# fusiyuan2010/CSC

Hardware: AMD Instinct MI355X
Metric: encode MB/s (10^6 input bytes / wall-clock) on enwik9 stand-in, -m3 -d64m; stream bit-exact vs reference (higher is better)
Workload: dtype u8/u32 (byte + 32-bit integer work; 12-bit probabilities, 64-bit range-coder low)

## Files before the change

### csc_amd/csrc/csc_host.cpp

```cpp
#include <hip/hip_runtime.h>
#include <chrono>

#include <math.h>
#include <stdio.h>
#include <stdlib.h>
#include <string.h>

#include <mutex>
#include <vector>

#include "../../include/csc_mi355x.h"
#include "csc_device.h"
#include "csc_enc_frame.h"
#include "csc_tables.h"

namespace cscmi {
hipError_t upload_tables();
void launch_frame_blocks(const FrameItem *items, FrameJob *jobs, FrameStatus *status, uint32_t nstreams, hipStream_t st);
void launch_init_state(EncState *S, hipStream_t st);
void launch_analyze(EncState *S, uint32_t chunk_size, const double *ent_coef, hipStream_t st);
void launch_encode_runs(int parser, EncState *S, const RunDesc *runs, uint32_t nruns, uint32_t reset_arena, hipStream_t st);
void launch_encode_eof(EncState *S, hipStream_t st);
void launch_encode_runs_multi(int parser, uint32_t nstreams, EncState *const *states, const RunDesc *const *runs,
                              const uint32_t *nruns, const uint32_t *reset, hipStream_t st);
// ... 1008 lines not shown
    HIPCHK(hipStreamSynchronize(e->stream));
    if (result) *result = e->h_small[0];
    return 0;
}
int CSCST_SetPos(CSCEncHandle p, uint32_t pos)
{
    EncInstance *e = (EncInstance *)p;
    if (!e) return -1;
    HIPCHK(hipSetDevice(e->device));
    HIPCHK(hipStreamSynchronize(e->stream));
    HIPCHK(hipMemcpy(&e->d_state->pos, &pos, sizeof(pos), hipMemcpyHostToDevice));
    return 0;
}
#endif

#ifdef CSCMI_TIMERS
void CSCMI_DebugTimers(CSCEncHandle p, uint64_t *out16)
{
    EncInstance *e = (EncInstance *)p;
    KernelStats ks;
    memset(&ks, 0, sizeof(ks));
    (void)hipSetDevice(e->device);
    (void)hipMemcpy(&ks, &e->d_state->stats, sizeof(ks), hipMemcpyDeviceToHost);
    for (int i = 0; i < 16; i++) out16[i] = ks.tm[i];
}

void CSCMI_DebugSetMask(CSCEncHandle p, uint64_t mask)
{
    EncInstance *e = (EncInstance *)p;
    (void)hipSetDevice(e->device);
    (void)hipMemcpy(&e->d_state->stats.trace[63][0], &mask, sizeof(mask), hipMemcpyHostToDevice);
}

void CSCMI_DebugTrace(CSCEncHandle p, uint64_t *out768)
{
    EncInstance *e = (EncInstance *)p;
    static KernelStats ks;
    memset(&ks, 0, sizeof(ks));
    (void)hipSetDevice(e->device);
    (void)hipMemcpy(&ks, &e->d_state->stats, sizeof(ks), hipMemcpyDeviceToHost);
    memcpy(out768, ks.trace, sizeof(ks.trace));
}
#endif

}
```

### csc_amd/csrc/csc_kernels_dp4.inc

```

constexpr uint32_t kD4Rec = 256;
constexpr uint32_t kD4CandEnt = kD4Rec * 4;
constexpr uint32_t kD4RefEnt = 256;
constexpr uint32_t kD4Ent = kD4CandEnt + kD4RefEnt;
constexpr uint32_t kD4LA = 48;
constexpr uint32_t kD4Waves = 12;
DEV uint32_t d4_role(uint32_t w)
{
    constexpr uint32_t roles[12] = { 0, 6, 7, 1, 8, 5, 4, 2, 8, 8, 9, 3 };
    return w < 12 ? roles[w] : 8u;
}
constexpr uint32_t kD4Requested = 0xFFFFFFFFu;
#ifndef D4_IDLE_MUL
#define D4_IDLE_MUL 1
#endif
constexpr int kD4IdleSleep = 4 * D4_IDLE_MUL;
constexpr uint32_t kD4RefreshAt = 32;
constexpr uint32_t kD4MaxGood = 16;
constexpr uint32_t kD6Ring = 128;
constexpr uint32_t kD6MRing = 64;
constexpr uint32_t kD4MultiMax = 768;

struct Dp4X {
    uint32_t sb_seq, sb_ack, quit, abort;
    uint32_t sb0, pos0, size, gen;
    uint32_t m_pos;
    uint32_t m_ids[2];
    uint32_t ins_head;
    uint32_t cmp_next, cmp_pause, cmp_idle[3], cmp_cur[3];
    uint32_t ev_seq, ev_s, ev_len, ev_ack;
    uint32_t ref_head;
    uint32_t rq_head, rq_tail;
    uint32_t lit_req, lit_from, lit_done;
    uint32_t rid[4];
    uint32_t io_w0, io_gen, io_state0, io_lp_int, io_lit_seq, io_rq_head, io_wnd_lo, io_wnd_hi, io_wnd_size, io_vld, io_good, io_plit_lo, io_plit_hi;
    alignas(16) uint32_t o_kind, o_end, o_a0l, o_a0code, o_a0eid, o_a0slot, o_fin_i0, o_fin_i1, o_lp_int, o_lit_seq, o_rq_head, o_err;
#ifdef CSCMI_TIMERS
    uint32_t stat[8];
    uint32_t wtm[52];
#endif
    uint32_t rq[16][2];
    raw_vec4 cand[kD4Rec];
    uint8_t hflag[kD4Rec];
    uint32_t rec_tag[kD4Rec], rec_hsum[kD4Rec], rec_a0d[kD4Rec], rec_len[kD4Rec][16];
    uint32_t rec_m32[kD4Rec][16];
    raw_vec4 ent[kD4Ent];
    uint32_t fwd[kD4Ent];
    alignas(512) uint16_t litp[4][kD4Rec];
    alignas(16) uint16_t tab[64][32];
    alignas(256) raw_vec4 lab[16];
    alignas(512) uint32_t tent[2][16][8];
    alignas(256) raw_vec4 ver[16];
    uint32_t lab_seq, win_seq;
    alignas(16) uint32_t dump[8];
    alignas(8) uint32_t e_prog[2]; uint32_t e_stop[2];
#ifdef CSCMI_TIMERS
    uint32_t dbgp[64], dbgq[64][8], dbgl[32];
    uint32_t dbg;
    uint32_t tr_win, tr_lo, tr_hi;
#endif
    uint32_t lenp_new[32];
    uint32_t lt_pub, lt_done;
    uint32_t lt_rec[kD6Ring];
    uint32_t mt_pub, mt_done;
    uint32_t mt_rec[kD6MRing][2];
    uint32_t hS[2], h_reset, hand[20];
};
struct EncLds4 { EncLds base; Dp4X x; CoderQ q; };
__shared__ EncLds4 g_lds4;

DEV uint32_t d4_tag(uint32_t gen, uint32_t p) { return ((gen << 13) | p) + 1u; }
DEV Dp4X *d4x(Sc &c) { return reinterpret_cast<Dp4X *>(c.X); }

DEV uint32_t d4_eq4(uint32_t x)
{
    const uint32_t z = ~(((x & 0x7F7F7F7Fu) + 0x7F7F7F7Fu) | x) & 0x80808080u;
    return (((z >> 7) * 0x01020408u) >> 24) & 0xFu;
}
DEV uint32_t d4_eq8(uint64_t x) { return d4_eq4((uint32_t)x) | (d4_eq4((uint32_t)(x >> 32)) << 4); }

DEV bool d4_spin(Sc &c, Dp4X *X, uint32_t &spins, uint32_t site)
{
    __builtin_amdgcn_s_sleep(1);
    if ((++spins & 1023u) == 0 && (spins > (kDpSpinLimit << 2) || lds_vload(&X->abort))) {
        if (!lds_vload(&X->abort)) lds_vstore(&X->abort, 0x40000000u | (site << 16) | (c.wv << 24) | (spins & 0xFFFFu));
        c.error = lds_vload(&X->abort);
        return false;
    }
    return true;
}
template <int LANE> DEV uint32_t d4_wrlane(uint32_t old, uint32_t val)
{
// ... 1128 lines not shown
        if (__ballot(ask) != 0) rq_head = UNI(d4_ask(__ballot(ask), rid_v, wpos, rq_head));
        if (__ballot(arrived) != 0) { lds_fence(); if (arrived) rid_v = fwv - 1; }
        const bool hard = lane < 4 && !arrived && age >= kD5HardAge && age < 0x80000000u;
        if (__builtin_expect(__ballot(hard) == 0, 1)) break;
        __builtin_amdgcn_s_sleep(1);
#ifdef CSCMI_TIMERS
        if (spins == 0 && lane == 0) atomicAdd(&X->stat[7], 1u);
#endif
        if ((++spins & 4095u) == 0 && (UNI(*(lds_vu32 *)&X->abort) || spins > (kDpSpinLimit << 2))) {
            if (!UNI(*(lds_vu32 *)&X->abort)) *(lds_vu32 *)&X->abort = 0x40100000u | (spins & 0xFFFFu);
            break;
        }
    }
    raw_vec4 r;
    r.x = rdlane(rid_v, 0) | (rdlane(rid_v, 1) << 16); r.y = rdlane(rid_v, 2) | (rdlane(rid_v, 3) << 16); r.z = rq_head; r.w = 0;
    return r;
}

__device__ __noinline__ void d5_spine()
{
    EncLds *L = &g_lds4.base;
    Dp4X *X = &g_lds4.x;
    const uint32_t lane = threadIdx.x & 63u;
    const uint32_t sb0 = UNI(X->sb0), size = UNI(X->size);
    const uint32_t w0 = UNI(X->io_w0), good = UNI(X->io_good);
    uint32_t lit_seq = UNI(X->io_lit_seq), rq_head = UNI(X->io_rq_head);
    const uint32_t aplimit = umin(kAPLimit, size - w0);
    const uint32_t sel_rid = lane < 4 ? 0x0C0C0100u + lane * 0x0202u : 0x0C0C0C0Cu;
#ifdef CSCMI_TIMERS
    const unsigned long long tsp = __builtin_readcyclecounter();
    unsigned long long t_first = 0, t_poll = 0, t_gen = 0, t_last = 0;
    uint32_t n_gen = 0;
#endif
    dp_fence();
    lit_seq++;
    d5_lit_guard(lit_seq);
    *(lds_vu32 *)&X->lit_from = umin(w0 + 8u, size);
    lds_fence();
    *(lds_vu32 *)&X->lit_req = lit_seq;
    uint32_t own_p = 0, own_bit = 0;
    const uint32_t own_pos = w0 + (lane >> 3);
    {
        const gu32 *p_lit = (const gu32 *)(((uint64_t)UNI(X->io_plit_hi) << 32) | UNI(X->io_plit_lo));
        const uint32_t b01 = (uint32_t)stage_load8(L->stage, umin(own_pos, size) + 15u);
        const uint32_t ctx = (sb0 + own_pos) ? (b01 & 0xFFu) : 0u, cc = ((b01 >> 8) & 0xFFu) | 0x100u;
        const uint32_t j = lane & 7u;
        own_bit = (cc >> (7u - j)) & 1u;
        if (own_pos < size) own_p = p_lit[ctx * 256u + (cc >> (8u - j))];
    }
    {
        const uint32_t lastwin = UNI(*(lds_vu32 *)&X->win_seq);
        uint32_t spins = 0;
        while (!(lds_vload(&X->e_stop[0]) == lastwin && lds_vload(&X->e_stop[1]) == lastwin)) {
            if ((++spins & 4095u) == 0 && (lds_vload(&X->abort) || spins > (kDpSpinLimit << 2))) { if (!lds_vload(&X->abort)) *(lds_vu32 *)&X->abort = 0x400F0000u; break; }
        }
        lds_fence();
    }
    d4_build_tables_inl();
    {
        uint32_t pr = L->p2b[(own_bit ? own_p : 4096u - own_p) >> 3];
        pr += (uint32_t)__shfl_xor((int)pr, 1);
        pr += (uint32_t)__shfl_xor((int)pr, 2);
        pr += (uint32_t)__shfl_xor((int)pr, 4);
        if ((lane & 7u) == 0 && own_pos < size) X->litp[lit_seq & 3u][own_pos & (kD4Rec - 1)] = (uint16_t)pr;
        lds_fence();
    }
    const uint32_t own_upto = w0 + 8u;
    uint32_t vz;
    asm volatile("v_mov_b32 %0, 0" : "=v"(vz));
    uint32_t vP = vz, vD = vz, vBS = (UNI(X->io_state0) << 16) | vz;
    uint32_t vI0, vI1;
    {
        uint32_t i0 = UNI(X->rid[0]) | (UNI(X->rid[1]) << 16), i1 = UNI(X->rid[2]) | (UNI(X->rid[3]) << 16);
        d5_forward_ids(X, lane, sel_rid, i0, i1);
        vI0 = i0 | vz; vI1 = i1 | vz;
    }
    uint32_t v_lp = UNI(X->io_lp_int) | vz, v_reach = vz;
    uint32_t refreshed = 0, have_new = 0;
    {
        const uint32_t lp0 = UNI(v_lp);
        if (lp0 < 96u) { d6_wait_match_trees(); d4_len_price_rebuild(X->lenp_new); have_new = 1; }
        raw_vec4 lb;
        lb.x = vP; lb.y = vBS | (lp0 < kD5Zone2 ? (lp0 + 1u) << 24 : 0u); lb.z = vI0; lb.w = vI1;
        *(lds_vvec4 *)&X->lab[0] = lb;
    }
    *(lds_vu32 *)&X->tent[0][1][0] = kD5Inf; *(lds_vu32 *)&X->tent[1][1][0] = kD5Inf; *(lds_vu32 *)&X->tent[1][2][0] = kD5Inf;
    { raw_vec4 z; z.x = z.y = z.z = z.w = 0; *(lds_vvec4 *)&X->ver[15] = z; }
    lds_fence();
    *(lds_vu32 *)&X->lab_seq = 1;
    const uint32_t win = UNI(*(lds_vu32 *)&X->win_seq) + 1u;
    const uint32_t winhi = (win & 0xFFFFu) << 16;
    lds_fence();
    *(lds_vu32 *)&X->win_seq = win;
#ifdef CSCMI_TIMERS
    const unsigned long long ts0 = __builtin_readcyclecounter();
    uint32_t n_straight = 0;
    unsigned long long *const TR = (unsigned long long *)(((uint64_t)UNI(X->tr_hi) << 32) | UNI(X->tr_lo));
    const bool tr_on = win == UNI(X->tr_win);
#endif
    uint32_t k = 0, kind = DP_CONT, end = 0, vnext = 0, lit_ok = own_upto, err = 0;
    uint32_t a0l = 1, a0code = 0, a0eid = 0, a0slot = 0, fI0 = 0, fI1 = 0;
    typedef volatile __attribute__((address_space(3))) uint8_t lds_vu8;
    const uint32_t f7 = lane & 7u, l16 = lane & 15u;
    const uint32_t mP = f7 == D5F_P ? ~0u : 0u, mBS = f7 == D5F_BS ? ~0u : 0u, mD = f7 == D5F_D ? ~0u : 0u, mTBV = f7 == D5F_TBV ? ~0u : 0u;
    const uint32_t shv = f7 == D5F_M32 ? 1u : 0u;
    const uint32_t c_left = f7 == D5F_LEFT ? ~0u : 0u;
    const uint32_t m_lsign = f7 == D5F_LEFT ? 0x80000000u : 0u;
    const uint32_t mlow = f7 == D5F_BS ? 0xFFFFu : ~0u;
    const uint32_t mI0 = f7 == D5F_I0 ? ~0u : 0u, mI1 = f7 == D5F_I1 ? ~0u : 0u, mM32 = f7 == D5F_M32 ? ~0u : 0u;
    auto lbl_pack = [&](uint32_t P, uint32_t D, uint32_t BS, uint32_t I0, uint32_t I1, uint32_t TBV, uint32_t M32, uint32_t LEFT) -> uint32_t {
        return (P & mP) | (BS & mBS) | (D & mD) | (I0 & mI0) | (I1 & mI1) | (TBV & mTBV) | (M32 & mM32) | (LEFT & c_left);
    };
    const uint32_t m_lab = 0u - ((0x001Bu >> l16) & 1u), m_log = 0u - ((0x0204u >> l16) & 1u);
    const uint32_t a_img = (uint32_t)(uintptr_t)(lds_vu8 *)&g_lds4;
    const uint32_t a_lab = a_img + (((uint32_t)(uintptr_t)(lds_vu8 *)&X->lab[0] - a_img) & m_lab);
    auto lds_at = [](uint32_t a) { return (lds_vu32 *)(uintptr_t)a; };
    static_assert(sizeof(((Dp4X *)nullptr)->lab) == 256 && sizeof(((Dp4X *)nullptr)->dump) >= 32, "label ring of 16 x 16 bytes (the store offset wraps at 256); eight dump words");
    const uint32_t r_log0 = (uint32_t)(uintptr_t)(lds_vu8 *)&L->fin2[0] - a_img, r_dump = (uint32_t)(uintptr_t)(lds_vu8 *)&X->dump[0] - a_img;
    const uint32_t st_inc = (16u & m_lab) | (8u & m_log);
    const uint32_t st_and = 255u | ~m_lab;
    const uint32_t w_lab = ((0x32010u >> (l16 * 4u)) & 0xFu) * 4u;
    const uint32_t w_log = (l16 >> 3) * 4u;
    auto st_seek = [&](uint32_t kk) -> uint32_t {
        const uint32_t o_lab = (kk & 15u) * 16u + w_lab, o_log = r_log0 + kk * 8u + w_log, o_dmp = r_dump + f7 * 4u;
        return (o_lab & m_lab) | (o_log & m_log) | (o_dmp & ~(m_lab | m_log));
    };
    uint64_t prog = 0;
    raw_vec4 V;
    uint32_t T0 = 0, T1 = 0, tree = 0;
    V.x = V.y = V.z = V.w = 0;
    static_assert(sizeof(((Dp4X *)nullptr)->ver) == 256 && sizeof(((Dp4X *)nullptr)->tent[0]) == 512 && sizeof(((Dp4X *)nullptr)->litp[0]) == 512, "ring sizes the address wraps assume");
    const uint32_t a_ver0 = (uint32_t)(uintptr_t)(lds_vu8 *)&X->ver[0], a_tent0 = (uint32_t)(uintptr_t)(lds_vu8 *)&X->tent[0][0][0];
    const uint32_t a_litp0 = (uint32_t)(uintptr_t)(lds_vu8 *)&X->litp[lit_seq & 3u][0];
// ... 316 lines not shown
                    bP = UNI(A.x); bBS = UNI(A.y); bD = UNI(A.z); bI0 = UNI(A.w); bI1 = UNI(*(lds_vu32 *)&X->tent[t & 1u][t & 15u][4]);
                }
                if (k >= 2) {
                    const raw_vec4 B = *(lds_vvec4 *)&X->tent[k & 1u][t & 15u][0];
                    const uint32_t qP = UNI(B.x), qBS = UNI(B.y), qD = UNI(B.z), qI0 = UNI(B.w), qI1 = UNI(*(lds_vu32 *)&X->tent[k & 1u][t & 15u][4]);
                    if (qP < bP || (qP == bP && (qBS & 0xFFFFu) < (bBS & 0xFFFFu))) { bP = qP; bD = qD; bBS = qBS; bI0 = qI0; bI1 = qI1; }
                }
                if (eP < bP) { bP = eP; bD = eD; bBS = eBS; bI0 = cI0; bI1 = cI1; }
                cP = bP; cD = bD; cBS = bBS; cI0 = bI0; cI1 = bI1;
                k++;
                raw_vec4 lb;
                lb.x = cP; lb.y = cBS | (refreshed << 31) | (lp_int < kD5Zone2 ? (lp_int + 1u) << 24 : 0u); lb.z = cI0; lb.w = cI1;
                *(lds_vvec4 *)&X->lab[k & 15u] = lb;
                L->fin2[k * 2u] = cD; L->fin2[k * 2u + 1u] = cBS;
#ifdef CSCMI_TIMERS
                if (k < 64) { X->dbgq[k][0] = cP; X->dbgq[k][5] = eP; X->dbgq[k][6] = 2; X->dbgq[k][7] = lp_int; }
#endif
                lds_fence();
                *(lds_vu32 *)&X->lab_seq = k + 1u;
            }
            vP = cP | vz; vD = cD | vz; vBS = cBS | vz; vI0 = cI0 | vz; vI1 = cI1 | vz; v_lp = lp_int | vz; v_reach = reach | vz;
            fI0 = cI0; fI1 = cI1;
            if (!out) pf_label();
#ifdef CSCMI_TIMERS
            t_gen += __builtin_readcyclecounter() - tg0;
#endif
            if (out) break;
        }
    }
#ifdef CSCMI_TIMERS
    const unsigned long long tse = __builtin_readcyclecounter();
    if (lane == 0) { atomicAdd(&X->wtm[13], (uint32_t)(tse - ts0) >> 4); atomicAdd(&X->wtm[14], n_straight); atomicAdd(&X->wtm[15], 1u);
        atomicAdd(&X->wtm[24], (uint32_t)(ts0 - tsp) >> 4); atomicAdd(&X->wtm[25], (uint32_t)t_first >> 4); atomicAdd(&X->wtm[26], (uint32_t)t_poll >> 4);
        atomicAdd(&X->wtm[27], (uint32_t)t_gen >> 4); atomicAdd(&X->wtm[28], n_gen); atomicAdd(&X->wtm[29], (uint32_t)(tse - t_last) >> 4); }
#endif
    lds_fence();
    *(lds_vu32 *)&X->lab_seq = kD5Stop;
    if (refreshed) { if (lane < 32) L->len_price[lane] = X->lenp_new[lane]; lds_fence(); }
    uint32_t f0 = kind == DP_EXIT_LIMIT ? fI0 : UNI(X->lab[end & 15u].z);
    uint32_t f1 = kind == DP_EXIT_LIMIT ? fI1 : UNI(X->lab[end & 15u].w);
    d5_forward_ids(X, lane, sel_rid, f0, f1);
    *(lds_vu32 *)&X->m_pos = w0 + end; *(lds_vu32 *)&X->m_ids[0] = f0; *(lds_vu32 *)&X->m_ids[1] = f1;
    {
        raw_vec4 o0, o1, o2;
        o0.x = kind; o0.y = end; o0.z = a0l; o0.w = a0code; o1.x = a0eid; o1.y = a0slot; o1.z = f0; o1.w = f1;
        o2.x = v_lp; o2.y = lit_seq; o2.z = rq_head; o2.w = err;
        *(lds_vvec4 *)&X->o_kind = o0; *(lds_vvec4 *)&X->o_a0eid = o1; *(lds_vvec4 *)&X->o_lp_int = o2;
    }
    lds_fence();
#ifdef CSCMI_TIMERS
    if (lane == 0) atomicAdd(&X->wtm[30], (uint32_t)(__builtin_readcyclecounter() - tse) >> 4);
#endif
}

DEV void d4_request(Sc &c, Dp4X *X, uint32_t id, uint32_t base, uint32_t &rq_head)
{
    if (rq_head - lds_vload(&X->rq_tail) >= 16u) return;
    X->rq[rq_head & 15u][0] = id;
    X->rq[rq_head & 15u][1] = base;
    X->fwd[id] = kD4Requested;
    rq_head++;
    lds_fence();
    lds_vstore(&X->rq_head, rq_head);
}

DEV bool d4_rebase_reps(Sc &c, Dp4X *X, uint32_t base, uint32_t &rq_head, bool wait)
{
// ... 315 lines not shown
        bool later = false;
        if (n > 1) {
#pragma unroll
            for (uint32_t j = 0; j < 4; j++) {
                if (j >= n) break;
                const D6Rec Rj = d6_rec(rdlane(w0, j << sh), rdlane(dist, j << sh));
                const uint32_t kj = d6_rec_lane(Rj, idx);
                const bool hit = kj != 0xFFu;
                if (hit && j < i) { prev = (j << sh) + kj; rank++; }
                later = later || (hit && j > i);
            }
        }
        uint32_t pnew = p_update(bit, pold);
        for (uint32_t d = 1; d < n && __ballot(rank >= d) != 0; d++) {
            const uint32_t v = (uint32_t)__builtin_amdgcn_ds_bpermute((int)(prev * 4u), (int)pnew);
            if (rank == d) { pold = v; pnew = p_update(bit, pold); }
        }
        c.L->P[on && !later ? idx : kPDumpE] = pnew;
        {
            const uint32_t kd = k - ((1u << sh) - 2u);
            const bool dir = i < n && kd < R.ndir;
            const uint32_t at = dir ? qpos + R.n_head + kd : qpos + k + (k >= R.n_head ? R.ndir : 0u);
            lds_vu32 *const slot_p = on || dir ? (lds_vu32 *)&g_lds4.q.e[at & (kCoderQ - 1)] : (lds_vu32 *)&g_lds4.q.pad;
            *slot_p = dir ? 0x40000000u | (kd ? R.dir1 : R.dir0) : 0x80000000u | (bit << 12) | pold;
        }
        lds_fence();
        mdone += n;
        lds_vstore(&X->mt_done, mdone);
#ifdef CSCMI_TIMERS
        if (lane == 0) { atomicAdd(&X->wtm[48], 1u); atomicAdd(&X->wtm[49], n); }
#endif
    }
    while (done != pub) {
        const uint32_t nlit = umin(pub - done, 16u), n_a = umin(nlit, 8u), n_b = nlit - n_a;
        const uint32_t lane = c.lane, i = lane >> 3, k = lane & 7u;
        const uint32_t rec_a = *(lds_vu32 *)&X->lt_rec[(done + i) & (kD6Ring - 1)], rec_b = *(lds_vu32 *)&X->lt_rec[(done + 8u + i) & (kD6Ring - 1)];
        const uint32_t cc_a = ((rec_a >> 8) & 0xFFu) | 0x100u, cc_b = ((rec_b >> 8) & 0xFFu) | 0x100u;
        const uint32_t bit_a = (cc_a >> (7u - k)) & 1u, bit_b = (cc_b >> (7u - k)) & 1u;
        const bool act_a = i < n_a, act_b = i < n_b;
        const uint32_t cell_a = act_a ? (rec_a & 0xFFu) * 256u + (cc_a >> (8u - k)) : 0x80000000u | lane;
        const uint32_t cell_b = act_b ? (rec_b & 0xFFu) * 256u + (cc_b >> (8u - k)) : 0x80000040u | lane;
        uint32_t pold_a = 0, pold_b = 0;
        if (act_a) pold_a = c.p_lit[cell_a];
        if (act_b) pold_b = c.p_lit[cell_b];
        uint32_t prev_a = 0, prev_b = 0;
        bool later_a = false, later_b = false;
#pragma unroll
        for (uint32_t j = 7; j >= 1; j--) {
            const uint32_t o = (uint32_t)__builtin_amdgcn_ds_bpermute((int)((lane - 8u * j) * 4u), (int)cell_a);
            prev_a = (i >= j && o == cell_a) ? j : prev_a;
            const uint32_t o2 = (uint32_t)__builtin_amdgcn_ds_bpermute((int)((lane + 8u * j) * 4u), (int)cell_a);
            later_a = later_a || (i + j < 8u && o2 == cell_a);
        }
        uint32_t from_a = 0;
        if (n_b) {
#pragma unroll
            for (uint32_t j = 7; j >= 1; j--) {
                const uint32_t o = (uint32_t)__builtin_amdgcn_ds_bpermute((int)((lane - 8u * j) * 4u), (int)cell_b);
                prev_b = (i >= j && o == cell_b) ? j : prev_b;
                const uint32_t o2 = (uint32_t)__builtin_amdgcn_ds_bpermute((int)((lane + 8u * j) * 4u), (int)cell_b);
                later_b = later_b || (i + j < 8u && o2 == cell_b);
            }
#pragma unroll
            for (uint32_t j = 0; j < 8; j++) {
                const uint32_t r = (i + j) & 7u;
                const uint32_t oa = (uint32_t)__builtin_amdgcn_ds_bpermute((int)((lane + 8u * j) * 4u), (int)cell_a);
// ... 81 lines not shown
    D6Cur tq;
    tq.lt_head = lds_vload(&X->lt_pub); tq.lt_seen = lds_vload(&X->lt_done); tq.mt_head = lds_vload(&X->mt_pub); tq.mt_seen = lds_vload(&X->mt_done);

    for (uint32_t i = 0; i < size;) {
        if (lds_vload(&X->abort)) { c.error = lds_vload(&X->abort); return; }
        TM_DECL;
        const uint32_t w0 = i;
        lds_vstore(&X->m_pos, i);
        if (ev_pending) {
            uint32_t spins = 0;
            while (lds_vload(&X->ev_ack) != ev_seq) if (!d4_spin(c, X, spins, 6)) return;
            lds_fence();
            gen = lds_vload(&X->gen);
            ev_pending = false;
        }
        TM_ADD(c, 0);
        {
            const uint32_t rs = w0 & (kD4Rec - 1);
            const uint32_t tg = *(lds_vu32 *)&X->rec_tag[rs], hs = *(lds_vu32 *)&X->rec_hsum[rs];
            const uint32_t rid_l = *(lds_vu32 *)&X->rid[lane & 3u];
            const raw_vec4 en = *(lds_vvec4 *)&X->ent[rid_l];
            const uint32_t wpos = sb0 + w0, off = wpos - en.y;
            const uint32_t mlow = (uint32_t)((((uint64_t)en.w << 32) | en.z) >> (off & 63u));
            const uint32_t bad = (off >> 6) | ((((off & 63u) + 1u) >> 6) & mlow) | ((umin(en.x - en.y - 1u, 0x7FFFFFFFu) - off) >> 31) | (((mlow & 3u) + 1u) >> 2);
            if (UNI(tg) == d4_tag(gen, w0) && (UNI(hs) & 0xFFu) == 0 && __ballot(bad != 0) == 0 && w0 + 1u < size && !D5FLAG(30)) {
                if (!d6_room(c, X, 16u, tq)) return;
                if (!d6_literal(c, X, stage_byte(c, sb0 + w0), tq)) return;
                TM_ADD(c, 4);
                c.st_find++;
                i++;
                continue;
            }
        }
        if (!d6_join(c, X, tq, true)) return;
        TM_ADD(c, 5);
        if (__builtin_expect(c.error != 0, 0)) { if (!lds_vload(&X->abort)) lds_vstore(&X->abort, c.error); return; }
        X->io_w0 = w0; X->io_gen = gen; X->io_state0 = c.state; X->io_lp_int = c.lp_rebuild_int; X->io_lit_seq = lit_seq; X->io_rq_head = rq_head;
        lds_fence();
#ifdef CSCMI_TIMERS
        if (D5DBG(32u) && c.lane < 32) X->dbgl[c.lane] = L->len_price[c.lane];
#endif
#ifdef CSCMI_TIMERS
        const bool d5_here = (lds_vload(&X->dbg) >> 8) == 0 || D5DBG(64u) || pos0 + w0 < (lds_vload(&X->dbg) >> 8) * 16u;
#else
        const bool d5_here = true;
#endif
#ifdef CSCMI_TIMERS
        if (kD5Split && !D5DBG(16u) && d5_here) d5_spine();
        else d4_window();
#else
        (void)d5_here;
        d5_spine();
#endif
#ifdef CSCMI_TIMERS
        if (D5DBG(128u) && pos0 + w0 + 1024u >= (lds_vload(&X->dbg) >> 8) * 16u) { for (int q = 0; q < 100; q++) __builtin_amdgcn_s_sleep(127); }
#endif
#ifdef CSCMI_TIMERS
        if (D5DBG(32u) && lds_vload(&X->o_end) < 150u && c.S->stats.trace[62][0] == 0
            && (!D5DBG(64u) || (pos0 + w0 < (lds_vload(&X->dbg) >> 8) * 16u && pos0 + w0 + 16u >= (lds_vload(&X->dbg) >> 8) * 16u))) {
            auto sig = [&]() -> uint32_t {
                uint32_t h = lds_vload(&X->o_kind) * 0x9E3779B1u + lds_vload(&X->o_end);
                h = h * 0x85EBCA6Bu + lds_vload(&X->o_a0l); h = h * 0x85EBCA6Bu + lds_vload(&X->o_a0code); h = h * 0x85EBCA6Bu + lds_vload(&X->o_lp_int);
                if (lds_vload(&X->o_kind) == DP_EXIT_MATCH) { h = h * 0x85EBCA6Bu + lds_vload(&X->o_a0slot); if (lds_vload(&X->o_a0code) > 4) h = h * 0x85EBCA6Bu + UNI(X->ent[lds_vload(&X->o_a0eid)].x); }
                { const uint32_t f0 = lds_vload(&X->o_fin_i0), f1 = lds_vload(&X->o_fin_i1);
                  h = h * 31u + UNI(X->ent[f0 & 0xFFFFu].x); h = h * 31u + UNI(X->ent[f0 >> 16].x); h = h * 31u + UNI(X->ent[f1 & 0xFFFFu].x); h = h * 31u + UNI(X->ent[f1 >> 16].x); }
                for (uint32_t t = lds_vload(&X->o_end); t;) {
                    const uint32_t b = UNI(L->fin2[t * 2u + 1u] & 0xFFFFu), d = UNI(L->fin2[t * 2u]);
                    h = (h ^ (t * 31u + d)) * 0x01000193u;
                    t = b;
                }
                return h;
            };
            auto sig2 = [&]() -> uint32_t {
                uint32_t h = 0;
                for (uint32_t q = 0; q < 32; q++) h = h * 31u + UNI(L->len_price[q]);
                return h;
            };
            auto snap = [&](unsigned long long *T) {
                uint32_t hf = 0, he = 0;
                for (uint32_t q = c.lane; q < kD4Ent; q += 64) { hf += X->fwd[q] * (q * 2u + 1u); const raw_vec4 e = X->ent[q]; he += (e.x * 3u + e.y * 5u + e.z * 7u + e.w * 11u) * (q * 2u + 1u); }
                for (int o = 32; o; o >>= 1) { hf += __shfl_xor(hf, o); he += __shfl_xor(he, o); }
                if (c.lane == 0) {
                    T[0] = hf; T[1] = he; T[2] = lds_vload(&X->ref_head); T[3] = lds_vload(&X->rq_head) | ((unsigned long long)lds_vload(&X->rq_tail) << 32);
                    T[4] = lds_vload(&X->lit_req) | ((unsigned long long)lds_vload(&X->lit_done) << 32); T[5] = lds_vload(&X->m_pos);
                    T[6] = lds_vload(&X->m_ids[0]) | ((unsigned long long)lds_vload(&X->m_ids[1]) << 32); T[7] = lds_vload(&X->gen) | ((unsigned long long)lds_vload(&X->ins_head) << 32);
// ... 221 lines not shown
        for (int q = 0; q < 8; q++) atomicAdd(&c.S->stats.tm[q], c.tm[q]);
#endif
    }
    lds_fence();
}
DEV void d4_master_call(Sc &c, uint32_t size)
{
    Dp4X *X = d4x(c);
    if (c.lane == 0) {
        X->hand[0] = c.wnd_curpos; X->hand[1] = c.stage_base; X->hand[2] = c.stage_end; X->hand[3] = c.pos;
        X->hand[5] = c.state; X->hand[6] = c.ctx; X->hand[7] = c.lp_rebuild_int; X->hand[8] = c.q_head; X->hand[9] = c.q_room; X->hand[10] = size;
    }
    lds_fence();
    d4_master_nl();
    c.wnd_curpos = lds_vload(&X->hand[0]); c.pos = lds_vload(&X->hand[3]); c.state = lds_vload(&X->hand[5]);
    c.ctx = lds_vload(&X->hand[6]); c.lp_rebuild_int = lds_vload(&X->hand[7]); c.q_head = lds_vload(&X->hand[8]); c.q_room = lds_vload(&X->hand[9]);
    const uint32_t err = lds_vload(&X->hand[11]);
    if (err && !c.error) c.error = err;
    c.st_find += lds_vload(&X->hand[12]); c.st_slide += lds_vload(&X->hand[13]); c.st_bt += lds_vload(&X->hand[14]);
    c.st_lit += lds_vload(&X->hand[15]); c.st_match += lds_vload(&X->hand[16]);
}

DEV void d4_init(Sc &c, uint32_t reset_arena)
{
    Dp4X *X = d4x(c);
    uint32_t *w = reinterpret_cast<uint32_t *>(X);
    const uint32_t nctl = (uint32_t)(offsetof(Dp4X, cand) / 4);
    for (uint32_t t = threadIdx.x; t < nctl; t += blockDim.x) w[t] = 0;
    for (uint32_t t = threadIdx.x; t < kD4Rec; t += blockDim.x) X->rec_tag[t] = 0;
    if (threadIdx.x < 3) X->cmp_idle[threadIdx.x] = 1;
    if (threadIdx.x < 2) { X->e_prog[threadIdx.x] = 0xFFFF0000u; X->e_stop[threadIdx.x] = 0; }
    if (threadIdx.x == 0) { X->lab_seq = 0; X->win_seq = 0; X->lt_pub = 0; X->lt_done = 0; X->mt_pub = 0; X->mt_done = 0; }
#ifdef CSCMI_TIMERS
    if (threadIdx.x == 0) { X->dbg = (uint32_t)c.S->stats.trace[63][0]; X->tr_win = (uint32_t)(c.S->stats.trace[63][0] >> 32);
        const uint64_t ta = (uint64_t)(uintptr_t)&c.S->stats.trace[0][0]; X->tr_lo = (uint32_t)ta; X->tr_hi = (uint32_t)(ta >> 32); }
#endif
    if (threadIdx.x < 4) (&g_lds4.q.pub)[threadIdx.x] = 0;
    if (threadIdx.x == 0) { X->hS[0] = (uint32_t)(uintptr_t)c.S; X->hS[1] = (uint32_t)((uint64_t)(uintptr_t)c.S >> 32); X->h_reset = reset_arena; }
}
DEV CoderQ *d4_coderq(Sc &c) { (void)c; return &g_lds4.q; }
DEV void d4_worker(Sc &c);
__device__ __noinline__ void d4_worker_nl()
{
    Dp4X *X = &g_lds4.x;
    Sc c;
    const uint64_t sp = ((uint64_t)lds_vload(&X->hS[1]) << 32) | lds_vload(&X->hS[0]);
    sc_load_regs(c, (EncState *)(uintptr_t)sp, &g_lds4.base);
    c.X = X;
    if (lds_vload(&X->h_reset)) c.arena_used = 0;
    c.bt_head = nullptr; c.bt_nodes = nullptr; c.bt_bits = 0; c.bt_size = 0; c.gmb = 0; c.fast_ht = true; c.pair_ok = 0;
    c.wv = UNI(threadIdx.x >> 6);
    d4_worker(c);
}
DEV void d4_worker_call(Sc &) { d4_worker_nl(); }

DEV void d4_coder(Sc &c)
{
    CoderQ *Q = &g_lds4.q;
    Dp4X *X = d4x(c);
    uint32_t tail = 0;
    for (;;) {
        uint32_t pub;
        while ((pub = lds_vload(&Q->pub)) == tail) {
            if (lds_vload(&X->quit)) {
                EncState *S = c.S;
                if (c.lane == 0) {
                    S->rc_low = c.rc_low; S->rc_range = c.rc_range; S->rc_cache = c.rc_cache; S->rc_cachesize = c.rc_cachesize;
// ... 23 lines not shown
            lds_vstore(&Q->tail, tail);
        }
#ifdef CSCMI_TIMERS
        if (c.lane == 0) { atomicAdd(&X->wtm[43], (uint32_t)(__builtin_readcyclecounter() - tc0) >> 4); atomicAdd(&X->wtm[44], tail - tail0); atomicAdd(&X->wtm[45], 1u); }
#endif
    }
}

DEV void d4_worker(Sc &c)
{
    c.wv = d4_role(c.wv);
    if (c.wv == 8) return;
    if (c.wv == 1) d4_inserter(c);
    else if (c.wv == 9) d6_trees(c);
    else if (c.wv == 4) d4_service(c);
    else if (c.wv == 5) d4_coder(c);
    else if (c.wv >= 6) d5_edges(c, c.wv - 6u);
    else d4_compare(c, c.wv == 2 ? 0u : 1u);
}
DEV void d4_quit(Sc &c)
{
    Dp4X *X = d4x(c);
    if (c.Q) {
        q_publish(c);
        uint32_t spins = 0;
        while (lds_vload(&c.Q->tail) != c.q_head) if (!d4_spin(c, X, spins, 11)) break;
    }
    dp_fence();
    lds_vstore(&X->quit, 1);
    if (!c.error && lds_vload(&X->abort)) c.error = lds_vload(&X->abort);
#ifdef CSCMI_TIMERS
    for (int q = 2; q < 8; q++) c.tm[8 + q] += lds_vload(&X->stat[q]);
    if (g_lds4.x.dbgl[31] && c.S->stats.trace[61][0] == 0 && c.lane < 4 && g_lds4.x.dbgq[c.lane][2]) { unsigned long long *T = c.S->stats.trace[60]; T[12 * 0 + c.lane * 3 + 0] = g_lds4.x.dbgq[c.lane][0] + ((unsigned long long)g_lds4.x.dbgq[c.lane][4] << 32); T[c.lane * 3 + 1] = g_lds4.x.dbgq[c.lane][1] + ((unsigned long long)g_lds4.x.dbgq[c.lane][3] << 32); T[c.lane * 3 + 2] = g_lds4.x.dbgq[c.lane][2]; c.S->stats.trace[61][0] = 1; }
    if (c.lane == 0) for (int q = 0; q < 52; q++) atomicAdd((unsigned long long *)&c.S->stats.trace[q / 12][q % 12], (unsigned long long)lds_vload(&X->wtm[q]));
#endif
}
```

Measured before the change: 3.059.

## Defer literal-tree join into spine so window setup overlaps literal pricing

The blocking d6_join wait on literal-table completion before each window is removed from the driver. Instead, the spine publishes the target literal head and does its table build, label seeding and window start first. Only after that does it wait on lt_done, so the literal pricing wave overlaps the spine's setup. It also adds a debug-only stress hook, and it risks ordering bugs if any setup step depended on completed literal tables.

```diff
diff --git a/csc_amd/csrc/csc_host.cpp b/csc_amd/csrc/csc_host.cpp
--- a/csc_amd/csrc/csc_host.cpp
+++ b/csc_amd/csrc/csc_host.cpp
@@ -1064,6 +1064,13 @@
     (void)hipMemcpy(&e->d_state->stats.trace[63][0], &mask, sizeof(mask), hipMemcpyHostToDevice);
 }
 
+void CSCMI_DebugSetStress(CSCEncHandle p, uint64_t word)
+{
+    EncInstance *e = (EncInstance *)p;
+    (void)hipSetDevice(e->device);
+    (void)hipMemcpy(&e->d_state->stats.trace[61][1], &word, sizeof(word), hipMemcpyHostToDevice);
+}
+
 void CSCMI_DebugTrace(CSCEncHandle p, uint64_t *out768)
 {
     EncInstance *e = (EncInstance *)p;
diff --git a/csc_amd/csrc/csc_kernels_dp4.inc b/csc_amd/csrc/csc_kernels_dp4.inc
--- a/csc_amd/csrc/csc_kernels_dp4.inc
+++ b/csc_amd/csrc/csc_kernels_dp4.inc
@@ -33,11 +33,11 @@
     uint32_t rq_head, rq_tail;
     uint32_t lit_req, lit_from, lit_done;
     uint32_t rid[4];
-    uint32_t io_w0, io_gen, io_state0, io_lp_int, io_lit_seq, io_rq_head, io_wnd_lo, io_wnd_hi, io_wnd_size, io_vld, io_good, io_plit_lo, io_plit_hi;
+    uint32_t io_w0, io_gen, io_state0, io_lp_int, io_lit_seq, io_rq_head, io_wnd_lo, io_wnd_hi, io_wnd_size, io_vld, io_good, io_plit_lo, io_plit_hi, io_lt_head;
     alignas(16) uint32_t o_kind, o_end, o_a0l, o_a0code, o_a0eid, o_a0slot, o_fin_i0, o_fin_i1, o_lp_int, o_lit_seq, o_rq_head, o_err;
 #ifdef CSCMI_TIMERS
     uint32_t stat[8];
-    uint32_t wtm[52];
+    uint32_t wtm[54];
 #endif
     uint32_t rq[16][2];
     raw_vec4 cand[kD4Rec];
@@ -58,6 +58,7 @@
     uint32_t dbgp[64], dbgq[64][8], dbgl[32];
     uint32_t dbg;
     uint32_t tr_win, tr_lo, tr_hi;
+    uint32_t stress;
 #endif
     uint32_t lenp_new[32];
     uint32_t lt_pub, lt_done;
@@ -1252,7 +1253,64 @@
     unsigned long long t_first = 0, t_poll = 0, t_gen = 0, t_last = 0;
     uint32_t n_gen = 0;
 #endif
-    dp_fence();
+    {
+        const uint32_t lastwin = UNI(*(lds_vu32 *)&X->win_seq);
+        uint32_t spins = 0;
+        while (!(lds_vload(&X->e_stop[0]) == lastwin && lds_vload(&X->e_stop[1]) == lastwin)) {
+            if ((++spins & 4095u) == 0 && (lds_vload(&X->abort) || spins > (kDpSpinLimit << 2))) { if (!lds_vload(&X->abort)) *(lds_vu32 *)&X->abort = 0x400F0000u; break; }
+        }
+        lds_fence();
+    }
+    d4_build_tables_inl();
+    uint32_t vz;
+    asm volatile("v_mov_b32 %0, 0" : "=v"(vz));
+    uint32_t vP = vz, vD = vz, vBS = (UNI(X->io_state0) << 16) | vz;
+    uint32_t v_lp = UNI(X->io_lp_int) | vz, v_reach = vz;
+    uint32_t refreshed = 0, have_new = 0;
+    if (UNI(v_lp) < 96u) { d6_wait_match_trees(); d4_len_price_rebuild(X->lenp_new); have_new = 1; }
+    uint32_t vI0, vI1;
+    {
+        uint32_t i0 = UNI(X->rid[0]) | (UNI(X->rid[1]) << 16), i1 = UNI(X->rid[2]) | (UNI(X->rid[3]) << 16);
+        d5_forward_ids(X, lane, sel_rid, i0, i1);
+        vI0 = i0 | vz; vI1 = i1 | vz;
+    }
+    {
+        const uint32_t lp0 = UNI(v_lp);
+        raw_vec4 lb;
+        lb.x = vP; lb.y = vBS | (lp0 < kD5Zone2 ? (lp0 + 1u) << 24 : 0u); lb.z = vI0; lb.w = vI1;
+        *(lds_vvec4 *)&X->lab[0] = lb;
+    }
+    *(lds_vu32 *)&X->tent[0][1][0] = kD5Inf; *(lds_vu32 *)&X->tent[1][1][0] = kD5Inf; *(lds_vu32 *)&X->tent[1][2][0] = kD5Inf;
+    { raw_vec4 z; z.x = z.y = z.z = z.w = 0; *(lds_vvec4 *)&X->ver[15] = z; }
+    lds_fence();
+    *(lds_vu32 *)&X->lab_seq = 1;
+    const uint32_t win = UNI(*(lds_vu32 *)&X->win_seq) + 1u;
+    const uint32_t winhi = (win & 0xFFFFu) << 16;
+    lds_fence();
+    *(lds_vu32 *)&X->win_seq = win;
+#ifdef CSCMI_TIMERS
+    const unsigned long long t_a = __builtin_readcyclecounter();
+#endif
+    uint32_t join_bad = 0;
+    {
+        const uint32_t want = UNI(X->io_lt_head);
+        uint32_t spins = 0;
+#ifdef CSCMI_TIMERS
+        if (lds_vload(&X->lt_done) != want && lane == 0) atomicAdd(&X->wtm[52], 1u);
+#endif
+        while (lds_vload(&X->lt_done) != want) {
+            __builtin_amdgcn_s_sleep(1);
+            if ((++spins & 1023u) == 0 && (lds_vload(&X->abort) || spins > (kDpSpinLimit << 2))) {
+                if (!lds_vload(&X->abort)) *(lds_vu32 *)&X->abort = 0x40120000u | (spins & 0xFFFFu);
+                join_bad = 1;
+                break;
+            }
+        }
+        dp_fence();
+    }
+#ifdef CSCMI_TIMERS
+    const unsigned long long t_j = __builtin_readcyclecounter();
+#endif
     lit_seq++;
     d5_lit_guard(lit_seq);
     *(lds_vu32 *)&X->lit_from = umin(w0 + 8u, size);
@@ -1268,15 +1326,7 @@
         own_bit = (cc >> (7u - j)) & 1u;
         if (own_pos < size) own_p = p_lit[ctx * 256u + (cc >> (8u - j))];
     }
-    {
-        const uint32_t lastwin = UNI(*(lds_vu32 *)&X->win_seq);
-        uint32_t spins = 0;
-        while (!(lds_vload(&X->e_stop[0]) == lastwin && lds_vload(&X->e_stop[1]) == lastwin)) {
-            if ((++spins & 4095u) == 0 && (lds_vload(&X->abort) || spins > (kDpSpinLimit << 2))) { if (!lds_vload(&X->abort)) *(lds_vu32 *)&X->abort = 0x400F0000u; break; }
-        }
-        lds_fence();
-    }
-    d4_build_tables_inl();
+    const uint32_t own_upto = w0 + 8u;
     {
         uint32_t pr = L->p2b[(own_bit ? own_p : 4096u - own_p) >> 3];
         pr += (uint32_t)__shfl_xor((int)pr, 1);
@@ -1285,40 +1335,13 @@
         if ((lane & 7u) == 0 && own_pos < size) X->litp[lit_seq & 3u][own_pos & (kD4Rec - 1)] = (uint16_t)pr;
         lds_fence();
     }
-    const uint32_t own_upto = w0 + 8u;
-    uint32_t vz;
-    asm volatile("v_mov_b32 %0, 0" : "=v"(vz));
-    uint32_t vP = vz, vD = vz, vBS = (UNI(X->io_state0) << 16) | vz;
-    uint32_t vI0, vI1;
-    {
-        uint32_t i0 = UNI(X->rid[0]) | (UNI(X->rid[1]) << 16), i1 = UNI(X->rid[2]) | (UNI(X->rid[3]) << 16);
-        d5_forward_ids(X, lane, sel_rid, i0, i1);
-        vI0 = i0 | vz; vI1 = i1 | vz;
-    }
-    uint32_t v_lp = UNI(X->io_lp_int) | vz, v_reach = vz;
-    uint32_t refreshed = 0, have_new = 0;
-    {
-        const uint32_t lp0 = UNI(v_lp);
-        if (lp0 < 96u) { d6_wait_match_trees(); d4_len_price_rebuild(X->lenp_new); have_new = 1; }
-        raw_vec4 lb;
-        lb.x = vP; lb.y = vBS | (lp0 < kD5Zone2 ? (lp0 + 1u) << 24 : 0u); lb.z = vI0; lb.w = vI1;
-        *(lds_vvec4 *)&X->lab[0] = lb;
-    }
-    *(lds_vu32 *)&X->tent[0][1][0] = kD5Inf; *(lds_vu32 *)&X->tent[1][1][0] = kD5Inf; *(lds_vu32 *)&X->tent[1][2][0] = kD5Inf;
-    { raw_vec4 z; z.x = z.y = z.z = z.w = 0; *(lds_vvec4 *)&X->ver[15] = z; }
-    lds_fence();
-    *(lds_vu32 *)&X->lab_seq = 1;
-    const uint32_t win = UNI(*(lds_vu32 *)&X->win_seq) + 1u;
-    const uint32_t winhi = (win & 0xFFFFu) << 16;
-    lds_fence();
-    *(lds_vu32 *)&X->win_seq = win;
 #ifdef CSCMI_TIMERS
     const unsigned long long ts0 = __builtin_readcyclecounter();
     uint32_t n_straight = 0;
     unsigned long long *const TR = (unsigned long long *)(((uint64_t)UNI(X->tr_hi) << 32) | UNI(X->tr_lo));
     const bool tr_on = win == UNI(X->tr_win);
 #endif
-    uint32_t k = 0, kind = DP_CONT, end = 0, vnext = 0, lit_ok = own_upto, err = 0;
+    uint32_t k = 0, kind = DP_CONT, end = 0, vnext = 0, lit_ok = own_upto, err = join_bad;
     uint32_t a0l = 1, a0code = 0, a0eid = 0, a0slot = 0, fI0 = 0, fI1 = 0;
     typedef volatile __attribute__((address_space(3))) uint8_t lds_vu8;
     const uint32_t f7 = lane & 7u, l16 = lane & 15u;
@@ -1701,7 +1724,8 @@
     const unsigned long long tse = __builtin_readcyclecounter();
     if (lane == 0) { atomicAdd(&X->wtm[13], (uint32_t)(tse - ts0) >> 4); atomicAdd(&X->wtm[14], n_straight); atomicAdd(&X->wtm[15], 1u);
         atomicAdd(&X->wtm[24], (uint32_t)(ts0 - tsp) >> 4); atomicAdd(&X->wtm[25], (uint32_t)t_first >> 4); atomicAdd(&X->wtm[26], (uint32_t)t_poll >> 4);
-        atomicAdd(&X->wtm[27], (uint32_t)t_gen >> 4); atomicAdd(&X->wtm[28], n_gen); atomicAdd(&X->wtm[29], (uint32_t)(tse - t_last) >> 4); }
+        atomicAdd(&X->wtm[27], (uint32_t)t_gen >> 4); atomicAdd(&X->wtm[28], n_gen); atomicAdd(&X->wtm[29], (uint32_t)(tse - t_last) >> 4);
+        atomicAdd(&X->wtm[50], (uint32_t)(t_a - tsp) >> 4); atomicAdd(&X->wtm[51], (uint32_t)(t_j - t_a) >> 4); }
 #endif
     lds_fence();
     *(lds_vu32 *)&X->lab_seq = kD5Stop;
@@ -2083,6 +2107,9 @@
 #endif
     }
     while (done != pub) {
+#ifdef CSCMI_TIMERS
+        if (lds_vload(&X->stress) & 1u) for (int q = 0; q < 4; q++) __builtin_amdgcn_s_sleep(127);
+#endif
         const uint32_t nlit = umin(pub - done, 16u), n_a = umin(nlit, 8u), n_b = nlit - n_a;
         const uint32_t lane = c.lane, i = lane >> 3, k = lane & 7u;
         const uint32_t rec_a = *(lds_vu32 *)&X->lt_rec[(done + i) & (kD6Ring - 1)], rec_b = *(lds_vu32 *)&X->lt_rec[(done + 8u + i) & (kD6Ring - 1)];
@@ -2230,25 +2257,25 @@
                 continue;
             }
         }
-        if (!d6_join(c, X, tq, true)) return;
+#ifdef CSCMI_TIMERS
+        const bool d5_here = (lds_vload(&X->dbg) >> 8) == 0 || D5DBG(64u) || pos0 + w0 < (lds_vload(&X->dbg) >> 8) * 16u;
+        const bool d5_split = kD5Split && !D5DBG(16u) && d5_here;
+        if (!d5_split) { if (!d6_join(c, X, tq, true)) return; }
+#endif
         TM_ADD(c, 5);
         if (__builtin_expect(c.error != 0, 0)) { if (!lds_vload(&X->abort)) lds_vstore(&X->abort, c.error); return; }
         X->io_w0 = w0; X->io_gen = gen; X->io_state0 = c.state; X->io_lp_int = c.lp_rebuild_int; X->io_lit_seq = lit_seq; X->io_rq_head = rq_head;
+        X->io_lt_head = tq.lt_head;
         lds_fence();
 #ifdef CSCMI_TIMERS
         if (D5DBG(32u) && c.lane < 32) X->dbgl[c.lane] = L->len_price[c.lane];
 #endif
 #ifdef CSCMI_TIMERS
-        const bool d5_here = (lds_vload(&X->dbg) >> 8) == 0 || D5DBG(64u) || pos0 + w0 < (lds_vload(&X->dbg) >> 8) * 16u;
-#else
-        const bool d5_here = true;
-#endif
-#ifdef CSCMI_TIMERS
-        if (kD5Split && !D5DBG(16u) && d5_here) d5_spine();
+        if (d5_split) { d5_spine(); tq.lt_seen = tq.lt_head; }
         else d4_window();
 #else
-        (void)d5_here;
         d5_spine();
+        tq.lt_seen = tq.lt_head;
 #endif
 #ifdef CSCMI_TIMERS
         if (D5DBG(128u) && pos0 + w0 + 1024u >= (lds_vload(&X->dbg) >> 8) * 16u) { for (int q = 0; q < 100; q++) __builtin_amdgcn_s_sleep(127); }
@@ -2536,7 +2563,7 @@
     if (threadIdx.x < 2) { X->e_prog[threadIdx.x] = 0xFFFF0000u; X->e_stop[threadIdx.x] = 0; }
     if (threadIdx.x == 0) { X->lab_seq = 0; X->win_seq = 0; X->lt_pub = 0; X->lt_done = 0; X->mt_pub = 0; X->mt_done = 0; }
 #ifdef CSCMI_TIMERS
-    if (threadIdx.x == 0) { X->dbg = (uint32_t)c.S->stats.trace[63][0]; X->tr_win = (uint32_t)(c.S->stats.trace[63][0] >> 32);
+    if (threadIdx.x == 0) { X->dbg = (uint32_t)c.S->stats.trace[63][0]; X->tr_win = (uint32_t)(c.S->stats.trace[63][0] >> 32); X->stress = (uint32_t)c.S->stats.trace[61][1];
         const uint64_t ta = (uint64_t)(uintptr_t)&c.S->stats.trace[0][0]; X->tr_lo = (uint32_t)ta; X->tr_hi = (uint32_t)(ta >> 32); }
 #endif
     if (threadIdx.x < 4) (&g_lds4.q.pub)[threadIdx.x] = 0;
@@ -2626,6 +2653,6 @@
 #ifdef CSCMI_TIMERS
     for (int q = 2; q < 8; q++) c.tm[8 + q] += lds_vload(&X->stat[q]);
     if (g_lds4.x.dbgl[31] && c.S->stats.trace[61][0] == 0 && c.lane < 4 && g_lds4.x.dbgq[c.lane][2]) { unsigned long long *T = c.S->stats.trace[60]; T[12 * 0 + c.lane * 3 + 0] = g_lds4.x.dbgq[c.lane][0] + ((unsigned long long)g_lds4.x.dbgq[c.lane][4] << 32); T[c.lane * 3 + 1] = g_lds4.x.dbgq[c.lane][1] + ((unsigned long long)g_lds4.x.dbgq[c.lane][3] << 32); T[c.lane * 3 + 2] = g_lds4.x.dbgq[c.lane][2]; c.S->stats.trace[61][0] = 1; }
-    if (c.lane == 0) for (int q = 0; q < 52; q++) atomicAdd((unsigned long long *)&c.S->stats.trace[q / 12][q % 12], (unsigned long long)lds_vload(&X->wtm[q]));
-#endif
-}
+    if (c.lane == 0) for (int q = 0; q < 54; q++) atomicAdd((unsigned long long *)&c.S->stats.trace[q / 12][q % 12], (unsigned long long)lds_vload(&X->wtm[q]));
+#endif
+}
```

New measurement: 3.078 (median of 6 runs). About the same (+0.6%).
